# taipingeric/yolo-v4-tf.keras

Measured on AMD Instinct MI355X. Metric: images/sec end-to-end predict() at 608x608 batch 32; conv MFMA %peak, higher is better.
Workload: dtype bf16

## Files before the change

### yolo-v4-tf.keras_amd/csrc/resblock.hip

```cpp
#include <type_traits>

#include "conv_chain.h"

#ifndef RB_ABL
#define RB_ABL 0
#endif
#ifndef RB_RES_LDS
#define RB_RES_LDS 0
#endif
#ifndef RB_ST_AUX
#define RB_ST_AUX 0
#endif
#ifndef RB_LATE
#define RB_LATE 1
#endif

namespace y4 {

#ifdef RB_TRACE
__device__ unsigned long long rb_trace_buf[3 * 8 * 16];
#define RB_TR_WG 8
#define RB_TR_T0 1
#define RB_POINT(P)                                                                                         \
    do {                                                                                                    \
        __builtin_amdgcn_sched_barrier(0);                                                                  \
        if (tr_on) asm volatile("s_memtime %0" : "=s"(tr_t[P]));                                            \
        __builtin_amdgcn_sched_barrier(0);                                                                  \
    } while (0)
#else
#define RB_POINT(P)
#endif

constexpr int RB_ACT = (RB_ABL & 2) ? Y4_ACT_LEAKY : Y4_ACT_MISH;
constexpr int RB_T = 16, RB_H = RB_T + 2, RB_WAVES = 8;

template <int C, int TY = RB_T> struct RbGeom {
    static constexpr int HR = TY + 2;
    static constexpr int HROWS = HR * RB_H;
    static constexpr int NFA = HR + (2 * HR + 15) / 16;
    static constexpr int CPR = C / 8;
    static constexpr int ROWB = C * 2 + 16;
    static constexpr int XT_PIECES = (HROWS * (CPR + 1) + 63) / 64;
    static constexpr int NF = C / 16;
    static constexpr int KS1 = C / 32;
    static constexpr int STEP_BYTES = 2 * NF * 1024;
    static constexpr int P = KS1 / 2;
    static constexpr int NSTEPS = 10 * P;
    static constexpr int RING = 4;
    static constexpr int PPW = STEP_BYTES / 1024 / RB_WAVES;
    static constexpr int AFF_BYTES = 4 * C * 4;
    static constexpr int AFF_PAD = (AFF_BYTES + 1023) / 1024 * 1024;
    static constexpr int BLOB_BYTES = AFF_PAD + NSTEPS * STEP_BYTES;
    static constexpr int L_AFF = 0, L_RING = AFF_PAD, L_XT = L_RING + RING * STEP_BYTES;
    static constexpr int XT_SLACK = XT_PIECES * 1024 - HROWS * (CPR + 1) * 16;
    static constexpr int LDS = L_XT + XT_PIECES * 1024 + (XT_SLACK >= TOUCH_LDS ? 0 : 1024);
    static constexpr int L_TOUCH = LDS - TOUCH_LDS;
    static constexpr int WN = NF / 4, WM = RB_WAVES / WN, MREP = TY / WM;
    static_assert(C != 64 || 2 * LDS <= 160 * 1024, "C = 64: two workgroups per compute unit (resblock_dispatch)");
    static_assert(LDS <= 160 * 1024 && MREP >= 1 && MREP * WM == TY && PPW >= 1 && PPW * RB_WAVES * 1024 == STEP_BYTES && NFA <= 3 * RB_WAVES,
                  "resblock geometry");
};

struct ResBlockK {
    const char* in;
    char* out;
    const char* blob;
    int in_cstride, in_coff, out_cstride, out_coff;
    unsigned in_bytes, out_bytes;
    int N, S;
    int tiles_x, tiles_per_img, ntiles;
    int t_begin, t_end;
    int touch;
};

template <int DT, int C, int TY>
__global__ __launch_bounds__(64 * RB_WAVES, C == 64 ? 4 : 2) void resblock_kernel(const ResBlockK p) {
    using E = Elem<DT>;
    using G = RbGeom<C, TY>;
    constexpr int PARTS = RB_T / TY;
    constexpr int ROWB = G::ROWB, CPR = G::CPR, NF = G::NF, MREP = G::MREP;
    extern __shared__ __attribute__((aligned(16))) char smem[];
    const int tid = threadIdx.x, lane = tid & 63, wave = __builtin_amdgcn_readfirstlane(tid >> 6);
    const int q = lane & 15, g = lane >> 4;
    const int wm = wave / G::WN, wn = wave - wm * G::WN;
    const float* const aff = (const float*)(smem + G::L_AFF);
    char* const XT = smem + G::L_XT;
    char* const ring = smem + G::L_RING;

    const int GR = gridDim.x, xcd = blockIdx.x & 7, bi = blockIdx.x >> 3;
    const int nb_x = (GR - xcd + 7) >> 3;
    const int span = p.t_end - p.t_begin;
    const int t_lo = p.t_begin + (int)((int64_t)span * xcd / 8), t_hi = p.t_begin + (int)((int64_t)span * (xcd + 1) / 8);
    int t = t_lo + bi;
    auto locate = [&](int u, int& n, int& y_out0, int& tx) {
        const int full = u / PARTS, part = u - full * PARTS;
        n = full / p.tiles_per_img;
        const int rem = full - n * p.tiles_per_img, ty = rem / p.tiles_x;
        tx = rem - ty * p.tiles_x;
        y_out0 = ty * RB_T + part * TY;
    };

    const __amdgpu_buffer_rsrc_t rb = make_rsrc(p.blob, G::BLOB_BYTES);
    const __amdgpu_buffer_rsrc_t rs_in = make_rsrc(p.in, p.in_bytes), rs_out = make_rsrc(p.out, p.out_bytes);
    if (p.touch != 0) weight_touch(rb, smem + G::L_TOUCH, 0, G::BLOB_BYTES, wave, RB_WAVES, lane);
    for (int u = wave; u < G::AFF_PAD / 1024; u += RB_WAVES)
        buffer_load16_lds(rb, smem + __builtin_amdgcn_readfirstlane(u * 1024), u * 1024 + lane * 16, 0);
    auto stage_w = [&](int st) {
        char* const dst = ring + (st & (G::RING - 1)) * G::STEP_BYTES;
#pragma unroll
        for (int k = 0; k < G::PPW; ++k) {
            const int u = wave + k * RB_WAVES;
            buffer_load16_lds(rb, dst + __builtin_amdgcn_readfirstlane(u * 1024), G::AFF_PAD + u * 1024 + lane * 16, st * G::STEP_BYTES);
        }
    };
    auto load_x = [&](int tile) {
        int n, yo, tx;
        locate(tile, n, yo, tx);
        const int y0 = yo - 1, x0 = tx * RB_T - 1;
        constexpr int SPR = CPR + 1, DSLOT = RB_WAVES * 64, DHP = DSLOT / SPR, DCH = DSLOT % SPR, DHY = DHP / RB_H, DHX = DHP % RB_H;
        static_assert(DCH + SPR - 1 < 2 * SPR && DHX + RB_H < 2 * RB_H, "one carry per step");
        int slot0 = wave * 64 + lane;
        asm volatile("" : "+v"(slot0));
        const int hp0 = slot0 / SPR;
        int ch = slot0 - hp0 * SPR, hy = hp0 / RB_H;
        int hx = hp0 - hy * RB_H;
        const int pix_b = p.in_cstride * 2, row_b = p.S * pix_b;
        int off = (((n * p.S + y0) * p.S + x0) * p.in_cstride + p.in_coff) * 2 + hy * row_b + hx * pix_b + ch * 16;
        const int d_off = DHY * row_b + DHX * pix_b + DCH * 16, c_ch = pix_b - SPR * 16, c_hx = row_b - RB_H * pix_b;
#pragma unroll
        for (int k = 0; k * RB_WAVES < G::XT_PIECES; ++k) {
            const int u = wave + k * RB_WAVES;
            if (u < G::XT_PIECES) {
                const bool ok = ch < CPR && hy < G::HR && (unsigned)(y0 + hy) < (unsigned)p.S && (unsigned)(x0 + hx) < (unsigned)p.S;
                const int off_x = (RB_ABL & 128) ? (off & ~63) + (lane & 3) * 16 : off;
                buffer_load16_lds(rs_in, XT + __builtin_amdgcn_readfirstlane(u * 1024), ok ? off_x : (int)0x80000000, 0);
            }
            ch += DCH; hx += DHX; hy += DHY; off += d_off;
            if (ch >= SPR) { ch -= SPR; hx += 1; off += c_ch; }
            if (hx >= RB_H) { hx -= RB_H; hy += 1; off += c_hx; }
        }
    };
    if (t < t_hi) { load_x(t); stage_w(0); stage_w(1); stage_w(2); if (RB_LATE) stage_w(3); }

#ifdef RB_TRACE
    int tr_i = 0;
    unsigned long long tr_t[16] = {0, 0, 0, 0, 0, 0, 0, 0, 0, 0, 0, 0, 0, 0, 0, 0};
#endif
    for (; t < t_hi; t += nb_x) {
        int n, y_out0, tx;
        locate(t, n, y_out0, tx);
#ifdef RB_TRACE
        const bool tr_on = TY == RB_T && C == RB_TRACE && blockIdx.x == RB_TR_WG && tr_i >= RB_TR_T0 && tr_i < RB_TR_T0 + 3;
#endif
        RB_POINT(0);
        wait_vmcnt_then_barrier<0>();
        RB_POINT(1);

        u32x4 res[MREP][2];
        constexpr bool RES_LDS = RB_RES_LDS && (C == 128 || RB_RES_LDS > 1);
        if (RES_LDS) {
#pragma unroll
            for (int i = 0; i < MREP; ++i)
#pragma unroll
                for (int c = 0; c < 2; ++c)
                    res[i][c] = *(const u32x4*)(XT + ((wm * MREP + i + 1) * RB_H + q + 1) * ROWB + chunk_channel(wn * 64, c, g) * 2);
            asm volatile("s_waitcnt lgkmcnt(0)\n\ts_barrier" ::: "memory");
        }

        auto phase_a = [&](auto nfr_c) {
            constexpr int NFR = decltype(nfr_c)::value;
            char* row[NFR];
            bool inside[NFR];
#pragma unroll
            for (int k = 0; k < NFR; ++k) {
                const int f = wave + k * RB_WAVES;
                int hy, hx;
                if (f < G::HR) { hy = f; hx = 1 + q; }
                else { const int pp = min((f - G::HR) * 16 + q, 2 * G::HR - 1); hy = pp >> 1; hx = (pp & 1) * (RB_H - 1); }
                const int r = hy * RB_H + hx;
                row[k] = XT + r * ROWB;
                const int gy = y_out0 - 1 + hy, gx = tx * RB_T - 1 + hx;
                inside[k] = (unsigned)gy < (unsigned)p.S && (unsigned)gx < (unsigned)p.S;
            }
            f32x4 acc[NFR][NF];
#pragma unroll
            for (int k = 0; k < NFR; ++k)
#pragma unroll
                for (int j = 0; j < NF; ++j) acc[k][j] = f32x4{0.f, 0.f, 0.f, 0.f};
#pragma unroll
            for (int s = 0; s < G::KS1; ++s) {
                u32x4 xf[NFR], wf[NF];
#pragma unroll
                for (int k = 0; k < NFR; ++k) xf[k] = *(const u32x4*)(row[k] + (s * 4 + g) * 16);
#pragma unroll
                for (int j = 0; j < NF; ++j) wf[j] = *(const u32x4*)(ring + (s >> 1) * G::STEP_BYTES + (((s & 1) * NF + j) * 64 + lane) * 16);
#pragma unroll
                for (int k = 0; k < NFR; ++k)
#pragma unroll
                    for (int j = 0; j < NF; ++j) Mma<DT>::run(acc[k][j], wf[j], xf[k]);
            }
#pragma unroll
            for (int c = 0; c < NF / 2; ++c) {
                float sc[8], sh[8];
#pragma unroll
                for (int h = 0; h < 8; h += 4) {
                    const int ch = chunk_channel(0, c, g) + h;
                    const f32x4 s4 = *(const f32x4*)(aff + ch), h4 = *(const f32x4*)(aff + C + ch);
#pragma unroll
                    for (int e = 0; e < 4; ++e) { sc[h + e] = s4[e]; sh[h + e] = h4[e]; }
                }
#pragma unroll
                for (int k = 0; k < NFR; ++k) {
                    float v[8];
                    bn_act4<true, RB_ACT>(acc[k][2 * c], sc, sh, v);
                    bn_act4<true, RB_ACT>(acc[k][2 * c + 1], sc + 4, sh + 4, v + 4);
                    u32x4 pk;
                    E::store_chunk(&pk, v);
                    if (!inside[k]) pk = u32x4{0u, 0u, 0u, 0u};
                    *(u32x4*)(row[k] + (4 * c + g) * 16) = pk;
                }
            }
        };
        if (!(RB_ABL & 1)) {
            if (wave + 2 * RB_WAVES < G::NFA) phase_a(std::integral_constant<int, 3>{});
            else if (wave + RB_WAVES < G::NFA) phase_a(std::integral_constant<int, 2>{});
            else if (wave < G::NFA) phase_a(std::integral_constant<int, 1>{});
        }
        RB_POINT(2);
        asm volatile("s_waitcnt lgkmcnt(0)\n\ts_barrier" ::: "memory");
        RB_POINT(3);

        {
            int pix[MREP];
#pragma unroll
            for (int i = 0; i < MREP; ++i) {
                const int gy = y_out0 + wm * MREP + i, gx = tx * RB_T + q;
                pix[i] = gy < p.S && gx < p.S ? (n * p.S + gy) * p.S + gx : -1;
            }
            auto load_res = [&]() {
#pragma unroll
                for (int i = 0; i < MREP; ++i) {
                    const int o = pix[i] < 0 ? (int)0x80000000 : (pix[i] * p.in_cstride + p.in_coff) * 2;
#pragma unroll
                    for (int c = 0; c < 2; ++c) res[i][c] = buffer_load16(rs_in, o + chunk_channel(wn * 64, c, g) * 2);
                }
            };
            if (!RB_LATE && !RES_LDS) load_res();
            constexpr int S0 = G::NSTEPS - 4, RES_LOADS = RES_LDS ? 0 : 2 * MREP;
            f32x4 acc[MREP][4];
#pragma unroll
            for (int i = 0; i < MREP; ++i)
#pragma unroll
                for (int j = 0; j < 4; ++j) acc[i][j] = f32x4{0.f, 0.f, 0.f, 0.f};
#pragma unroll
            for (int st = RB_LATE ? 4 : 3; st <= G::P + 3; ++st) stage_w(st);
            const char* const xbase = XT + ((wm * MREP) * RB_H + q) * ROWB + g * 16;
            u32x4 xf[2][MREP], wf[2][4];
            auto read_frags = [&](int buf, int st, int kk) {
                if ((RB_ABL & 32) && st > G::P) return;
                const int ks = st - G::P;
                const int cb = ks / 9, tap = ks - cb * 9;
                const int ky = tap / 3, kx = tap - ky * 3;
                const char* const wst = ring + (st & (G::RING - 1)) * G::STEP_BYTES;
#pragma unroll
                for (int i = 0; i < MREP; ++i) {
                    xf[buf][i] = *(const u32x4*)(xbase + ((i + ky) * RB_H + kx) * ROWB + (cb * 8 + kk * 4) * 16);
                }
#pragma unroll
                for (int j = 0; j < 4; ++j) wf[buf][j] = *(const u32x4*)(wst + ((kk * NF + wn * 4 + j) * 64 + lane) * 16);
            };
            auto mma = [&](int buf) {
#pragma unroll
                for (int i = 0; i < MREP; ++i)
#pragma unroll
                    for (int j = 0; j < 4; ++j)
                        Mma<DT>::run(acc[i][j], wf[buf][j], xf[buf][i]);
            };
            RB_POINT(4);
            read_frags(0, G::P, 0);
#pragma unroll
            for (int st = G::P; st < G::NSTEPS; ++st) {
                if (st == G::P + 3 * G::P) RB_POINT(5);
                if (st == G::P + 6 * G::P) RB_POINT(6);
                if (RB_LATE && !RES_LDS && st == S0) load_res();
                read_frags(1, st, 1);
                __builtin_amdgcn_sched_barrier(0);
                mma(0);
                __builtin_amdgcn_sched_barrier(0);
                if (st + 1 < G::NSTEPS) {
                    constexpr int LAST = G::NSTEPS - 1;
                    const int younger = (st + 3 < LAST ? st + 3 : LAST) - (st + 1);
                    const int extra = RB_LATE && st >= S0 && st <= S0 + 2 ? RES_LOADS : 0;
                    static_assert(S0 > G::P && 2 * G::PPW + RES_LOADS < 64, "window of the residual's loads");
                    if (RB_ABL & 64) asm volatile("s_waitcnt vmcnt(0)" ::: "memory");
                    else wait_vmcnt_lgkm_then_barrier_n<2 * G::PPW + RES_LOADS>(younger == 0 ? 0 : (younger >= 2 ? 2 : 1) * G::PPW + extra);
                    if (!(RB_ABL & 4) && st + 4 < G::NSTEPS) stage_w(st + 4);
                    read_frags(0, st + 1, 0);
                    __builtin_amdgcn_sched_barrier(0);
                }
                mma(1);
                __builtin_amdgcn_sched_barrier(0);
            }
            RB_POINT(7);
            asm volatile("s_waitcnt lgkmcnt(0)\n\ts_barrier" ::: "memory");
            RB_POINT(8);
            if constexpr (RB_LATE && !RES_LDS) {
#pragma unroll
                for (int i = 0; i < MREP; ++i)
#pragma unroll
                    for (int c = 0; c < 2; ++c) asm volatile("" : "+v"(res[i][c]));
            }
            const bool more = t + nb_x < t_hi;
            if (more) { if (!(RB_ABL & 8)) load_x(t + nb_x); stage_w(0); stage_w(1); stage_w(2); if (RB_LATE) stage_w(3); }
            RB_POINT(9);
            float sc3[16], sh3[16];
#pragma unroll
            for (int c = 0; c < 2; ++c)
#pragma unroll
                for (int h = 0; h < 8; h += 4) {
                    const int ch = chunk_channel(wn * 64, c, g) + h;
                    const f32x4 s4 = *(const f32x4*)(aff + 2 * C + ch), h4 = *(const f32x4*)(aff + 3 * C + ch);
#pragma unroll
                    for (int e = 0; e < 4; ++e) { sc3[c * 8 + h + e] = s4[e]; sh3[c * 8 + h + e] = h4[e]; }
                }
#pragma unroll
            for (int i = 0; i < MREP; ++i) {
                float v[16];
#pragma unroll
                for (int j = 0; j < 4; ++j) bn_act4<true, RB_ACT>(acc[i][j], sc3 + j * 4, sh3 + j * 4, v + j * 4);
                const int o = pix[i] < 0 ? (int)0x80000000 : (pix[i] * p.out_cstride + p.out_coff) * 2;
#pragma unroll
                for (int c = 0; c < 2; ++c) {
                    float rv[8];
                    E::load_chunk(&res[i][c], rv);
#pragma unroll
                    for (int e = 0; e < 8; ++e) v[c * 8 + e] += rv[e];
                    u32x4 pk;
                    E::store_chunk(&pk, v + c * 8);
                    if (!(RB_ABL & 16) || pk[0] == 0x12345678u) buffer_store16<RB_ST_AUX>(rs_out, pk, o + chunk_channel(wn * 64, c, g) * 2);
                }
            }
        }
        RB_POINT(10);
#ifdef RB_TRACE
        if (tr_on && lane == 0) {
#pragma unroll
            for (int k = 0; k < 11; ++k) rb_trace_buf[((tr_i - RB_TR_T0) * 8 + wave) * 16 + k] = tr_t[k];
        }
        ++tr_i;
#endif
    }
}

#ifdef RB_TRACE
}
extern "C" int y4_rb_trace_read(unsigned long long* dst) {
    return (int)hipMemcpyFromSymbol(dst, HIP_SYMBOL(y4::rb_trace_buf), sizeof(unsigned long long) * 3 * 8 * 16);
}
namespace y4 {
#endif

bool resblock_supported(int dtype, int c) { return dtype != Y4_F32 && (c == 128 || c == 64); }
size_t resblock_blob_bytes(int c) { return c == 128 ? RbGeom<128>::BLOB_BYTES : RbGeom<64>::BLOB_BYTES; }

template <int DT, int C, int TY>
static int resblock_run(const ResBlockK& k, int slots, hipStream_t stream) {
    int grid = slots;
    const int span = k.t_end - k.t_begin;
    if (grid > ((span + 7) & ~7)) grid = (span + 7) & ~7;
    if (grid < 8) grid = 8;
    constexpr int lds = RbGeom<C, TY>::LDS;
    static PerDeviceOnce once;
    if (const uint64_t bit = once.due()) {
        Y4_CHECK_HIP(hipFuncSetAttribute((const void*)resblock_kernel<DT, C, TY>, hipFuncAttributeMaxDynamicSharedMemorySize, lds));
        once.mark(bit);
    }
    hipLaunchKernelGGL((resblock_kernel<DT, C, TY>), dim3(grid), dim3(64 * RB_WAVES), lds, stream, k);
    Y4_CHECK_HIP(hipGetLastError());
    return Y4_OK;
}

static bool rb_parts_enabled() {
    static const bool on = [] { const char* e = getenv("Y4_RB_PARTS"); return !(e && e[0] == '0'); }();
    return on;
}

template <int DT, int C>
static int resblock_dispatch(ResBlockK& k, hipStream_t stream) {
    static int n_cus[64] = {0};
    int dev = 0;
    Y4_CHECK_HIP(hipGetDevice(&dev));
    if (n_cus[dev & 63] == 0) {
        int v = 0;
        Y4_CHECK_HIP(hipDeviceGetAttribute(&v, hipDeviceAttributeMultiprocessorCount, dev));
        n_cus[dev & 63] = v > 0 ? v : 256;
    }
    const int slots = (n_cus[dev & 63] & ~7) * (C == 64 ? 2 : 1);
    constexpr int MAXP = C == 128 ? 4 : 2;
    const int full = k.ntiles / slots * slots, rem = k.ntiles - full;
    int parts = 1;
    if (rb_parts_enabled() && rem > 0)
        for (int pp = 2; pp <= MAXP; pp *= 2)
            if (rem * pp <= slots) parts = pp;
    if (parts == 1) {
        k.t_begin = 0; k.t_end = k.ntiles;
        return resblock_run<DT, C, RB_T>(k, slots, stream);
    }
    if (full > 0) {
        k.t_begin = 0; k.t_end = full;
        if (int r = resblock_run<DT, C, RB_T>(k, slots, stream)) return r;
    }
    k.t_begin = full * parts; k.t_end = k.ntiles * parts;
    if (parts == 2) return resblock_run<DT, C, RB_T / 2>(k, slots, stream);
    if constexpr (MAXP >= 4) return resblock_run<DT, C, RB_T / 4>(k, slots, stream);
    return Y4_EINVAL;
}

int resblock_launch(int dtype, int c, const void* in, int n, int side, int in_cstride, int in_coff, const void* blob, void* out,
                    int out_cstride, int out_coff, hipStream_t stream) {
    Y4_REQUIRE(resblock_supported(dtype, c), Y4_EINVAL, "resblock: dtype %d / %d channels not supported", dtype, c);
    Y4_REQUIRE(in && blob && out && n > 0 && side > 0, Y4_EINVAL, "resblock: null pointer / empty batch");
    Y4_REQUIRE(in_cstride % 8 == 0 && in_coff % 8 == 0 && out_cstride % 8 == 0 && out_coff % 8 == 0, Y4_EINVAL,
               "resblock: views not 16-byte aligned");
    const int64_t in_bytes = (int64_t)n * side * side * in_cstride * 2;
    const int64_t out_bytes = (int64_t)n * side * side * out_cstride * 2;
    Y4_REQUIRE(in_bytes < (1ll << 31) && out_bytes < (1ll << 31), Y4_EINVAL,
               "resblock: input (%lld B) or output (%lld B) exceeds the 2 GiB buffer-descriptor range", (long long)in_bytes, (long long)out_bytes);
    ResBlockK k{};
    k.in = (const char*)in; k.out = (char*)out; k.blob = (const char*)blob;
    k.in_cstride = in_cstride; k.in_coff = in_coff; k.out_cstride = out_cstride; k.out_coff = out_coff;
    k.in_bytes = (unsigned)in_bytes; k.out_bytes = (unsigned)out_bytes;
    k.N = n; k.S = side;
    k.touch = weight_touch_enabled() ? 1 : 0;
    k.tiles_x = (side + RB_T - 1) / RB_T; k.tiles_per_img = k.tiles_x * k.tiles_x; k.ntiles = n * k.tiles_per_img;
    if (c == 128) return dtype == Y4_BF16 ? resblock_dispatch<Y4_BF16, 128>(k, stream) : resblock_dispatch<Y4_F16, 128>(k, stream);
    return dtype == Y4_BF16 ? resblock_dispatch<Y4_BF16, 64>(k, stream) : resblock_dispatch<Y4_F16, 64>(k, stream);
}

template <int DT>
__global__ void rb_pack_frag_kernel(const float* __restrict__ w, typename Elem<DT>::type* __restrict__ out, int cout, int cin, int kk) {
    const int nrep = cout / 16, cbs = cin / 32, total = cout * cin * kk;
    for (int idx = blockIdx.x * blockDim.x + threadIdx.x; idx < total; idx += gridDim.x * blockDim.x) {
        const int e = idx & 7, lane = (idx >> 3) & 63, r = idx >> 9;
        const int j = r % nrep, s = r / nrep;
        const int step = s >> 1, cb64 = step / kk, tap = step - cb64 * kk, cb = cb64 * 2 + (s & 1);
        const int i = lane & 15, gg = lane >> 4;
        const int ch = ((j >> 1) * 4 + (i >> 2)) * 8 + (j & 1) * 4 + (i & 3);
        const int ci = 32 * cb + 8 * gg + e;
        out[idx] = Elem<DT>::st(w[((int64_t)ch * cin + ci) * kk + tap]);
    }
}
__global__ void rb_affine_kernel(const float* s1, const float* h1, const float* s3, const float* h3, float* dst, int c) {
    const int i = blockIdx.x * blockDim.x + threadIdx.x;
    if (i < c) { dst[i] = s1[i]; dst[c + i] = h1[i]; dst[2 * c + i] = s3[i]; dst[3 * c + i] = h3[i]; }
}

int pack_resblock(int dtype, int c, const float* w1, const float* scale1, const float* shift1, const float* w3, const float* scale3,
                  const float* shift3, void* blob, hipStream_t stream) {
    Y4_REQUIRE(resblock_supported(dtype, c) && w1 && w3 && scale1 && shift1 && scale3 && shift3 && blob, Y4_EINVAL, "pack_resblock: bad argument");
    const int w1_bytes = c * c * 2, aff_pad = (4 * c * 4 + 1023) / 1024 * 1024;
    char* b = (char*)blob;
    if (dtype == Y4_BF16) {
        hipLaunchKernelGGL(rb_pack_frag_kernel<Y4_BF16>, dim3((c * c + 255) / 256), dim3(256), 0, stream, w1, (uint16_t*)(b + aff_pad), c, c, 1);
        hipLaunchKernelGGL(rb_pack_frag_kernel<Y4_BF16>, dim3((9 * c * c + 255) / 256), dim3(256), 0, stream, w3, (uint16_t*)(b + aff_pad + w1_bytes), c, c, 9);
    } else {
        hipLaunchKernelGGL(rb_pack_frag_kernel<Y4_F16>, dim3((c * c + 255) / 256), dim3(256), 0, stream, w1, (_Float16*)(b + aff_pad), c, c, 1);
        hipLaunchKernelGGL(rb_pack_frag_kernel<Y4_F16>, dim3((9 * c * c + 255) / 256), dim3(256), 0, stream, w3, (_Float16*)(b + aff_pad + w1_bytes), c, c, 9);
    }
    hipLaunchKernelGGL(rb_affine_kernel, dim3(1), dim3(128), 0, stream, scale1, shift1, scale3, shift3, (float*)b, c);
    Y4_CHECK_HIP(hipGetLastError());
    return Y4_OK;
}

}
```

Baseline: 5923.

## Rewrite fused resblock kernel with 19x19 tiles, 4 waves, resident weights

Rewrites the fused 1x1+3x3 residual-block kernel. Tiles grow to 19x19 outputs with 4 waves and one workgroup per CU. The 1x1 weights, and for C=64 also the 3x3 weights, now stay resident in LDS. For C=128 the 3x3 weights stream from global memory into a register ring instead of an LDS staging ring with barriers. It also drops the tile-split tail dispatch, the weight-touch prefetch, the ablation flags and the trace instrumentation. The intent is to cut per-step barriers and LDS weight traffic and to lower halo overhead per output, at the cost of lower occupancy and more register pressure.

```diff
diff --git a/yolo-v4-tf.keras_amd/csrc/resblock.hip b/yolo-v4-tf.keras_amd/csrc/resblock.hip
--- a/yolo-v4-tf.keras_amd/csrc/resblock.hip
+++ b/yolo-v4-tf.keras_amd/csrc/resblock.hip
@@ -2,63 +2,55 @@
 
 #include "conv_chain.h"
 
-#ifndef RB_ABL
-#define RB_ABL 0
+#ifndef RB_WD
+#define RB_WD 4
 #endif
-#ifndef RB_RES_LDS
-#define RB_RES_LDS 0
-#endif
-#ifndef RB_ST_AUX
-#define RB_ST_AUX 0
-#endif
-#ifndef RB_LATE
-#define RB_LATE 1
-#endif
 
 namespace y4 {
 
-#ifdef RB_TRACE
-__device__ unsigned long long rb_trace_buf[3 * 8 * 16];
-#define RB_TR_WG 8
-#define RB_TR_T0 1
-#define RB_POINT(P)                                                                                         \
-    do {                                                                                                    \
-        __builtin_amdgcn_sched_barrier(0);                                                                  \
-        if (tr_on) asm volatile("s_memtime %0" : "=s"(tr_t[P]));                                            \
-        __builtin_amdgcn_sched_barrier(0);                                                                  \
-    } while (0)
-#else
-#define RB_POINT(P)
-#endif
-
-constexpr int RB_ACT = (RB_ABL & 2) ? Y4_ACT_LEAKY : Y4_ACT_MISH;
-constexpr int RB_T = 16, RB_H = RB_T + 2, RB_WAVES = 8;
-
-template <int C, int TY = RB_T> struct RbGeom {
-    static constexpr int HR = TY + 2;
-    static constexpr int HROWS = HR * RB_H;
-    static constexpr int NFA = HR + (2 * HR + 15) / 16;
+template <int I, int N, class F> __device__ __forceinline__ void rb_static_for(F&& f) {
+    if constexpr (I < N) {
+        f(std::integral_constant<int, I>{});
+        rb_static_for<I + 1, N>(f);
+    }
+}
+
+__device__ __forceinline__ u32x4 buffer_load16_so(__amdgpu_buffer_rsrc_t rsrc, int voffset, int soffset) {
+    return __builtin_amdgcn_raw_buffer_load_b128(rsrc, voffset, soffset, 0);
+}
+
+constexpr int RB_T = 19, RB_H = RB_T + 2, RB_WAVES = 4;
+constexpr int RB_HP = RB_H * RB_H;
+constexpr int RB_NFA = (RB_HP + 15) / 16;
+constexpr int RB_NPO = RB_T * RB_T;
+constexpr int RB_NFO = (RB_NPO + 15) / 16;
+
+template <int C> struct RbGeom {
+    static constexpr int NF = C / 16;
+    static constexpr int KS1 = C / 32, KS3 = 9 * KS1;
     static constexpr int CPR = C / 8;
-    static constexpr int ROWB = C * 2 + 16;
-    static constexpr int XT_PIECES = (HROWS * (CPR + 1) + 63) / 64;
-    static constexpr int NF = C / 16;
-    static constexpr int KS1 = C / 32;
-    static constexpr int STEP_BYTES = 2 * NF * 1024;
-    static constexpr int P = KS1 / 2;
-    static constexpr int NSTEPS = 10 * P;
-    static constexpr int RING = 4;
-    static constexpr int PPW = STEP_BYTES / 1024 / RB_WAVES;
+    static constexpr int SPR = CPR + 2, ROWB = SPR * 16;
+    static constexpr int EXTRA = C == 64 ? 192 : 0, RSTR = RB_H * ROWB + EXTRA;
+    static constexpr int RSPR = RSTR / 16;
+    static constexpr int XT_SLOTS = RB_H * RSPR + (RB_NFA * 16 - RB_HP) * SPR;
     static constexpr int AFF_BYTES = 4 * C * 4;
     static constexpr int AFF_PAD = (AFF_BYTES + 1023) / 1024 * 1024;
-    static constexpr int BLOB_BYTES = AFF_PAD + NSTEPS * STEP_BYTES;
-    static constexpr int L_AFF = 0, L_RING = AFF_PAD, L_XT = L_RING + RING * STEP_BYTES;
-    static constexpr int XT_SLACK = XT_PIECES * 1024 - HROWS * (CPR + 1) * 16;
-    static constexpr int LDS = L_XT + XT_PIECES * 1024 + (XT_SLACK >= TOUCH_LDS ? 0 : 1024);
-    static constexpr int L_TOUCH = LDS - TOUCH_LDS;
-    static constexpr int WN = NF / 4, WM = RB_WAVES / WN, MREP = TY / WM;
-    static_assert(C != 64 || 2 * LDS <= 160 * 1024, "C = 64: two workgroups per compute unit (resblock_dispatch)");
-    static_assert(LDS <= 160 * 1024 && MREP >= 1 && MREP * WM == TY && PPW >= 1 && PPW * RB_WAVES * 1024 == STEP_BYTES && NFA <= 3 * RB_WAVES,
-                  "resblock geometry");
+    static constexpr int W1_BYTES = C * C * 2, W3_BYTES = 9 * C * C * 2;
+    static constexpr int BLOB_BYTES = AFF_PAD + W1_BYTES + W3_BYTES;
+    static constexpr bool W3_LDS = C == 64;
+    static constexpr int L_W1 = AFF_PAD, L_W3 = AFF_PAD + W1_BYTES;
+    static constexpr int L_XT = AFF_PAD + W1_BYTES + (W3_LDS ? W3_BYTES : 0);
+    static constexpr int RES_PIECES = L_XT / 1024;
+    static constexpr int XT_PIECES = (XT_SLOTS + 63) / 64;
+    static constexpr int LDS = L_XT + XT_PIECES * 1024;
+    static constexpr int WF = C == 128 ? 2 : 4, WP = C == 128 ? RB_NFO : (RB_NFO + RB_WAVES - 1) / RB_WAVES;
+    static constexpr int WD = W3_LDS ? 2 : RB_WD;
+    static constexpr int S_RES = C == 128 ? KS3 - 12 : 0;
+    static constexpr int NST = WP * (WF / 2);
+    static_assert(L_XT % 1024 == 0 && EXTRA % 16 == 0 && LDS <= 160 * 1024, "resblock LDS layout");
+    static_assert(WF * (C == 128 ? RB_WAVES : 1) == NF && WP * (C == 128 ? 1 : RB_WAVES) >= RB_NFO && RB_NFA % RB_WAVES == 0,
+                  "resblock wave split");
+    static_assert(WD >= 2 && WD <= KS3, "weight ring depth");
 };
 
 struct ResBlockK {
@@ -69,133 +61,95 @@
     unsigned in_bytes, out_bytes;
     int N, S;
     int tiles_x, tiles_per_img, ntiles;
-    int t_begin, t_end;
-    int touch;
 };
 
-template <int DT, int C, int TY>
-__global__ __launch_bounds__(64 * RB_WAVES, C == 64 ? 4 : 2) void resblock_kernel(const ResBlockK p) {
+template <int DT, int C>
+__global__ __launch_bounds__(64 * RB_WAVES, 1) void resblock_kernel(const ResBlockK p) {
     using E = Elem<DT>;
-    using G = RbGeom<C, TY>;
-    constexpr int PARTS = RB_T / TY;
-    constexpr int ROWB = G::ROWB, CPR = G::CPR, NF = G::NF, MREP = G::MREP;
+    using G = RbGeom<C>;
+    constexpr int ROWB = G::ROWB, RSTR = G::RSTR, CPR = G::CPR, SPR = G::SPR, NF = G::NF, WF = G::WF, WP = G::WP, WD = G::WD;
     extern __shared__ __attribute__((aligned(16))) char smem[];
     const int tid = threadIdx.x, lane = tid & 63, wave = __builtin_amdgcn_readfirstlane(tid >> 6);
     const int q = lane & 15, g = lane >> 4;
-    const int wm = wave / G::WN, wn = wave - wm * G::WN;
-    const float* const aff = (const float*)(smem + G::L_AFF);
+    const float* const aff = (const float*)smem;
+    const char* const W1 = smem + G::L_W1;
+    const char* const W3L = smem + G::L_W3;
     char* const XT = smem + G::L_XT;
-    char* const ring = smem + G::L_RING;
 
     const int GR = gridDim.x, xcd = blockIdx.x & 7, bi = blockIdx.x >> 3;
     const int nb_x = (GR - xcd + 7) >> 3;
-    const int span = p.t_end - p.t_begin;
-    const int t_lo = p.t_begin + (int)((int64_t)span * xcd / 8), t_hi = p.t_begin + (int)((int64_t)span * (xcd + 1) / 8);
+    const int t_lo = (int)((int64_t)p.ntiles * xcd / 8), t_hi = (int)((int64_t)p.ntiles * (xcd + 1) / 8);
     int t = t_lo + bi;
-    auto locate = [&](int u, int& n, int& y_out0, int& tx) {
-        const int full = u / PARTS, part = u - full * PARTS;
-        n = full / p.tiles_per_img;
-        const int rem = full - n * p.tiles_per_img, ty = rem / p.tiles_x;
-        tx = rem - ty * p.tiles_x;
-        y_out0 = ty * RB_T + part * TY;
+    auto locate = [&](int u, int& n, int& y0, int& x0) {
+        n = u / p.tiles_per_img;
+        const int rem = u - n * p.tiles_per_img, ty = rem / p.tiles_x;
+        y0 = ty * RB_T;
+        x0 = (rem - ty * p.tiles_x) * RB_T;
     };
 
     const __amdgpu_buffer_rsrc_t rb = make_rsrc(p.blob, G::BLOB_BYTES);
     const __amdgpu_buffer_rsrc_t rs_in = make_rsrc(p.in, p.in_bytes), rs_out = make_rsrc(p.out, p.out_bytes);
-    if (p.touch != 0) weight_touch(rb, smem + G::L_TOUCH, 0, G::BLOB_BYTES, wave, RB_WAVES, lane);
-    for (int u = wave; u < G::AFF_PAD / 1024; u += RB_WAVES)
+    for (int u = wave; u < G::RES_PIECES; u += RB_WAVES)
         buffer_load16_lds(rb, smem + __builtin_amdgcn_readfirstlane(u * 1024), u * 1024 + lane * 16, 0);
-    auto stage_w = [&](int st) {
-        char* const dst = ring + (st & (G::RING - 1)) * G::STEP_BYTES;
-#pragma unroll
-        for (int k = 0; k < G::PPW; ++k) {
-            const int u = wave + k * RB_WAVES;
-            buffer_load16_lds(rb, dst + __builtin_amdgcn_readfirstlane(u * 1024), G::AFF_PAD + u * 1024 + lane * 16, st * G::STEP_BYTES);
+    auto load_x = [&](int tile) {
+        int n, y0, x0;
+        locate(tile, n, y0, x0);
+        const int pix_b = p.in_cstride * 2;
+        const int base = (((n * p.S + y0 - 1) * p.S + x0 - 1) * p.in_cstride + p.in_coff) * 2;
+        for (int u = wave; u < G::XT_PIECES; u += RB_WAVES) {
+            const int slot = u * 64 + lane, hy = slot / G::RSPR, r = slot - hy * G::RSPR, hx = r / SPR, ch = r - hx * SPR;
+            const bool ok = ch < CPR && hx < RB_H && hy < RB_H && (unsigned)(y0 - 1 + hy) < (unsigned)p.S && (unsigned)(x0 - 1 + hx) < (unsigned)p.S;
+            buffer_load16_lds(rs_in, XT + __builtin_amdgcn_readfirstlane(u * 1024), ok ? base + (hy * p.S + hx) * pix_b + ch * 16 : (int)0x80000000, 0);
         }
     };
-    auto load_x = [&](int tile) {
-        int n, yo, tx;
-        locate(tile, n, yo, tx);
-        const int y0 = yo - 1, x0 = tx * RB_T - 1;
-        constexpr int SPR = CPR + 1, DSLOT = RB_WAVES * 64, DHP = DSLOT / SPR, DCH = DSLOT % SPR, DHY = DHP / RB_H, DHX = DHP % RB_H;
-        static_assert(DCH + SPR - 1 < 2 * SPR && DHX + RB_H < 2 * RB_H, "one carry per step");
-        int slot0 = wave * 64 + lane;
-        asm volatile("" : "+v"(slot0));
-        const int hp0 = slot0 / SPR;
-        int ch = slot0 - hp0 * SPR, hy = hp0 / RB_H;
-        int hx = hp0 - hy * RB_H;
-        const int pix_b = p.in_cstride * 2, row_b = p.S * pix_b;
-        int off = (((n * p.S + y0) * p.S + x0) * p.in_cstride + p.in_coff) * 2 + hy * row_b + hx * pix_b + ch * 16;
-        const int d_off = DHY * row_b + DHX * pix_b + DCH * 16, c_ch = pix_b - SPR * 16, c_hx = row_b - RB_H * pix_b;
-#pragma unroll
-        for (int k = 0; k * RB_WAVES < G::XT_PIECES; ++k) {
-            const int u = wave + k * RB_WAVES;
-            if (u < G::XT_PIECES) {
-                const bool ok = ch < CPR && hy < G::HR && (unsigned)(y0 + hy) < (unsigned)p.S && (unsigned)(x0 + hx) < (unsigned)p.S;
-                const int off_x = (RB_ABL & 128) ? (off & ~63) + (lane & 3) * 16 : off;
-                buffer_load16_lds(rs_in, XT + __builtin_amdgcn_readfirstlane(u * 1024), ok ? off_x : (int)0x80000000, 0);
-            }
-            ch += DCH; hx += DHX; hy += DHY; off += d_off;
-            if (ch >= SPR) { ch -= SPR; hx += 1; off += c_ch; }
-            if (hx >= RB_H) { hx -= RB_H; hy += 1; off += c_hx; }
+    if (t < t_hi) load_x(t);
+
+    const int wfrag0 = G::W3_LDS ? 0 : wave * WF;
+    const int w3_off = G::L_W3 + (wfrag0 * 64 + lane) * 16;
+    auto fetch_w = [&](u32x4 (&w)[WF], int s) {
+#pragma unroll
+        for (int j = 0; j < WF; ++j) {
+            if constexpr (G::W3_LDS) w[j] = *(const u32x4*)(smem + w3_off + (s * NF + j) * 1024);
+            else w[j] = buffer_load16_so(rb, w3_off, (s * NF + j) * 1024);
         }
     };
-    if (t < t_hi) { load_x(t); stage_w(0); stage_w(1); stage_w(2); if (RB_LATE) stage_w(3); }
-
-#ifdef RB_TRACE
-    int tr_i = 0;
-    unsigned long long tr_t[16] = {0, 0, 0, 0, 0, 0, 0, 0, 0, 0, 0, 0, 0, 0, 0, 0};
-#endif
-    for (; t < t_hi; t += nb_x) {
-        int n, y_out0, tx;
-        locate(t, n, y_out0, tx);
-#ifdef RB_TRACE
-        const bool tr_on = TY == RB_T && C == RB_TRACE && blockIdx.x == RB_TR_WG && tr_i >= RB_TR_T0 && tr_i < RB_TR_T0 + 3;
-#endif
-        RB_POINT(0);
-        wait_vmcnt_then_barrier<0>();
-        RB_POINT(1);
-
-        u32x4 res[MREP][2];
-        constexpr bool RES_LDS = RB_RES_LDS && (C == 128 || RB_RES_LDS > 1);
-        if (RES_LDS) {
-#pragma unroll
-            for (int i = 0; i < MREP; ++i)
-#pragma unroll
-                for (int c = 0; c < 2; ++c)
-                    res[i][c] = *(const u32x4*)(XT + ((wm * MREP + i + 1) * RB_H + q + 1) * ROWB + chunk_channel(wn * 64, c, g) * 2);
-            asm volatile("s_waitcnt lgkmcnt(0)\n\ts_barrier" ::: "memory");
-        }
-
-        auto phase_a = [&](auto nfr_c) {
-            constexpr int NFR = decltype(nfr_c)::value;
-            char* row[NFR];
-            bool inside[NFR];
-#pragma unroll
-            for (int k = 0; k < NFR; ++k) {
-                const int f = wave + k * RB_WAVES;
-                int hy, hx;
-                if (f < G::HR) { hy = f; hx = 1 + q; }
-                else { const int pp = min((f - G::HR) * 16 + q, 2 * G::HR - 1); hy = pp >> 1; hx = (pp & 1) * (RB_H - 1); }
-                const int r = hy * RB_H + hx;
-                row[k] = XT + r * ROWB;
-                const int gy = y_out0 - 1 + hy, gx = tx * RB_T - 1 + hx;
-                inside[k] = (unsigned)gy < (unsigned)p.S && (unsigned)gx < (unsigned)p.S;
-            }
-            f32x4 acc[NFR][NF];
-#pragma unroll
-            for (int k = 0; k < NFR; ++k)
+    const int pf0 = G::W3_LDS ? wave * WP : 0;
+
+    for (bool first = true; t < t_hi; t += nb_x, first = false) {
+        int n, y0, x0;
+        locate(t, n, y0, x0);
+        if (first) wait_vmcnt_then_barrier<0>();
+        else wait_vmcnt_then_barrier<G::NST>();
+        u32x4 wr[WD][WF];
+#pragma unroll
+        for (int s = 0; s < WD - 1; ++s) fetch_w(wr[s], s);
+
+        {
+            constexpr int NA = RB_NFA / RB_WAVES;
+            char* row[NA];
+            bool inside[NA];
+            int qa = q;
+            asm volatile("" : "+v"(qa));
+#pragma unroll
+            for (int k = 0; k < NA; ++k) {
+                const int hp = (wave + k * RB_WAVES) * 16 + qa, hy = hp / RB_H, hx = hp - hy * RB_H;
+                row[k] = XT + hy * RSTR + hx * ROWB;
+                inside[k] = hp < RB_HP && (unsigned)(y0 - 1 + hy) < (unsigned)p.S && (unsigned)(x0 - 1 + hx) < (unsigned)p.S;
+            }
+            f32x4 acc[NA][NF];
+#pragma unroll
+            for (int k = 0; k < NA; ++k)
 #pragma unroll
                 for (int j = 0; j < NF; ++j) acc[k][j] = f32x4{0.f, 0.f, 0.f, 0.f};
 #pragma unroll
             for (int s = 0; s < G::KS1; ++s) {
-                u32x4 xf[NFR], wf[NF];
-#pragma unroll
-                for (int k = 0; k < NFR; ++k) xf[k] = *(const u32x4*)(row[k] + (s * 4 + g) * 16);
-#pragma unroll
-                for (int j = 0; j < NF; ++j) wf[j] = *(const u32x4*)(ring + (s >> 1) * G::STEP_BYTES + (((s & 1) * NF + j) * 64 + lane) * 16);
-#pragma unroll
-                for (int k = 0; k < NFR; ++k)
+                u32x4 xf[NA], wf[NF];
+#pragma unroll
+                for (int k = 0; k < NA; ++k) xf[k] = *(const u32x4*)(row[k] + (s * 4 + g) * 16);
+#pragma unroll
+                for (int j = 0; j < NF; ++j) wf[j] = *(const u32x4*)(W1 + ((s * NF + j) * 64 + lane) * 16);
+#pragma unroll
+                for (int k = 0; k < NA; ++k)
 #pragma unroll
                     for (int j = 0; j < NF; ++j) Mma<DT>::run(acc[k][j], wf[j], xf[k]);
             }
@@ -210,183 +164,103 @@
                     for (int e = 0; e < 4; ++e) { sc[h + e] = s4[e]; sh[h + e] = h4[e]; }
                 }
 #pragma unroll
-                for (int k = 0; k < NFR; ++k) {
+                for (int k = 0; k < NA; ++k) {
                     float v[8];
-                    bn_act4<true, RB_ACT>(acc[k][2 * c], sc, sh, v);
-                    bn_act4<true, RB_ACT>(acc[k][2 * c + 1], sc + 4, sh + 4, v + 4);
+                    bn_act4<true, Y4_ACT_MISH>(acc[k][2 * c], sc, sh, v);
+                    bn_act4<true, Y4_ACT_MISH>(acc[k][2 * c + 1], sc + 4, sh + 4, v + 4);
                     u32x4 pk;
                     E::store_chunk(&pk, v);
                     if (!inside[k]) pk = u32x4{0u, 0u, 0u, 0u};
                     *(u32x4*)(row[k] + (4 * c + g) * 16) = pk;
                 }
             }
+        }
+        asm volatile("s_waitcnt lgkmcnt(0)\n\ts_barrier" ::: "memory");
+
+        int xrow[WP];
+#pragma unroll
+        for (int i = 0; i < WP; ++i) {
+            const int pp = (pf0 + i) * 16 + q, pc = min(pp, RB_NPO - 1), oy = pc / RB_T, ox = pc - oy * RB_T;
+            xrow[i] = oy * RSTR + ox * ROWB + g * 16;
+        }
+        auto pix = [&](int i) {
+            int qq = q;
+            asm volatile("" : "+v"(qq));
+            const int pp = (pf0 + i) * 16 + qq, oy = pp / RB_T, ox = pp - oy * RB_T, gy = y0 + oy, gx = x0 + ox;
+            return ((pp < RB_NPO) & (gy < p.S) & (gx < p.S)) ? (n * p.S + gy) * p.S + gx : -1;
         };
-        if (!(RB_ABL & 1)) {
-            if (wave + 2 * RB_WAVES < G::NFA) phase_a(std::integral_constant<int, 3>{});
-            else if (wave + RB_WAVES < G::NFA) phase_a(std::integral_constant<int, 2>{});
-            else if (wave < G::NFA) phase_a(std::integral_constant<int, 1>{});
-        }
-        RB_POINT(2);
+        auto xoff = [](int s) constexpr {
+            const int cb = s / 18, r = s - cb * 18, tap = r >> 1, ky = tap / 3, kx = tap - ky * 3;
+            return ky * RSTR + kx * ROWB + (cb * 8 + (r & 1) * 4) * 16;
+        };
+        f32x4 acc[WP][WF];
+#pragma unroll
+        for (int i = 0; i < WP; ++i)
+#pragma unroll
+            for (int j = 0; j < WF; ++j) acc[i][j] = f32x4{0.f, 0.f, 0.f, 0.f};
+        u32x4 xf[WP];
+#pragma unroll
+        for (int i = 0; i < WP; ++i) xf[i] = *(const u32x4*)(XT + xrow[i]);
+        constexpr int NRES = WF / 2;
+        u32x4 res[WP][NRES];
+        rb_static_for<0, G::KS3>([&](auto sc) __attribute__((always_inline)) {
+            constexpr int s = decltype(sc)::value;
+            if constexpr (s + WD - 1 < G::KS3) fetch_w(wr[(s + WD - 1) % WD], s + WD - 1);
+            if constexpr (s == G::S_RES) {
+#pragma unroll
+                for (int i = 0; i < WP; ++i) {
+                    const int pi = pix(i), o = pi < 0 ? (int)0x80000000 : (pi * p.in_cstride + p.in_coff) * 2;
+#pragma unroll
+                    for (int c = 0; c < NRES; ++c) res[i][c] = buffer_load16(rs_in, o + chunk_channel(0, wfrag0 / 2 + c, g) * 2);
+                }
+            }
+            const u32x4(&w)[WF] = wr[s % WD];
+#pragma unroll
+            for (int i = 0; i < WP; ++i) {
+#pragma unroll
+                for (int j = 0; j < WF; ++j) Mma<DT>::run(acc[i][j], w[j], xf[i]);
+                if constexpr (s + 1 < G::KS3) xf[i] = *(const u32x4*)(XT + xrow[i] + xoff(s + 1));
+            }
+            __builtin_amdgcn_sched_barrier(0);
+        });
         asm volatile("s_waitcnt lgkmcnt(0)\n\ts_barrier" ::: "memory");
-        RB_POINT(3);
-
-        {
-            int pix[MREP];
-#pragma unroll
-            for (int i = 0; i < MREP; ++i) {
-                const int gy = y_out0 + wm * MREP + i, gx = tx * RB_T + q;
-                pix[i] = gy < p.S && gx < p.S ? (n * p.S + gy) * p.S + gx : -1;
-            }
-            auto load_res = [&]() {
-#pragma unroll
-                for (int i = 0; i < MREP; ++i) {
-                    const int o = pix[i] < 0 ? (int)0x80000000 : (pix[i] * p.in_cstride + p.in_coff) * 2;
-#pragma unroll
-                    for (int c = 0; c < 2; ++c) res[i][c] = buffer_load16(rs_in, o + chunk_channel(wn * 64, c, g) * 2);
-                }
-            };
-            if (!RB_LATE && !RES_LDS) load_res();
-            constexpr int S0 = G::NSTEPS - 4, RES_LOADS = RES_LDS ? 0 : 2 * MREP;
-            f32x4 acc[MREP][4];
-#pragma unroll
-            for (int i = 0; i < MREP; ++i)
-#pragma unroll
-                for (int j = 0; j < 4; ++j) acc[i][j] = f32x4{0.f, 0.f, 0.f, 0.f};
-#pragma unroll
-            for (int st = RB_LATE ? 4 : 3; st <= G::P + 3; ++st) stage_w(st);
-            const char* const xbase = XT + ((wm * MREP) * RB_H + q) * ROWB + g * 16;
-            u32x4 xf[2][MREP], wf[2][4];
-            auto read_frags = [&](int buf, int st, int kk) {
-                if ((RB_ABL & 32) && st > G::P) return;
-                const int ks = st - G::P;
-                const int cb = ks / 9, tap = ks - cb * 9;
-                const int ky = tap / 3, kx = tap - ky * 3;
-                const char* const wst = ring + (st & (G::RING - 1)) * G::STEP_BYTES;
-#pragma unroll
-                for (int i = 0; i < MREP; ++i) {
-                    xf[buf][i] = *(const u32x4*)(xbase + ((i + ky) * RB_H + kx) * ROWB + (cb * 8 + kk * 4) * 16);
-                }
-#pragma unroll
-                for (int j = 0; j < 4; ++j) wf[buf][j] = *(const u32x4*)(wst + ((kk * NF + wn * 4 + j) * 64 + lane) * 16);
-            };
-            auto mma = [&](int buf) {
-#pragma unroll
-                for (int i = 0; i < MREP; ++i)
-#pragma unroll
-                    for (int j = 0; j < 4; ++j)
-                        Mma<DT>::run(acc[i][j], wf[buf][j], xf[buf][i]);
-            };
-            RB_POINT(4);
-            read_frags(0, G::P, 0);
-#pragma unroll
-            for (int st = G::P; st < G::NSTEPS; ++st) {
-                if (st == G::P + 3 * G::P) RB_POINT(5);
-                if (st == G::P + 6 * G::P) RB_POINT(6);
-                if (RB_LATE && !RES_LDS && st == S0) load_res();
-                read_frags(1, st, 1);
-                __builtin_amdgcn_sched_barrier(0);
-                mma(0);
-                __builtin_amdgcn_sched_barrier(0);
-                if (st + 1 < G::NSTEPS) {
-                    constexpr int LAST = G::NSTEPS - 1;
-                    const int younger = (st + 3 < LAST ? st + 3 : LAST) - (st + 1);
-                    const int extra = RB_LATE && st >= S0 && st <= S0 + 2 ? RES_LOADS : 0;
-                    static_assert(S0 > G::P && 2 * G::PPW + RES_LOADS < 64, "window of the residual's loads");
-                    if (RB_ABL & 64) asm volatile("s_waitcnt vmcnt(0)" ::: "memory");
-                    else wait_vmcnt_lgkm_then_barrier_n<2 * G::PPW + RES_LOADS>(younger == 0 ? 0 : (younger >= 2 ? 2 : 1) * G::PPW + extra);
-                    if (!(RB_ABL & 4) && st + 4 < G::NSTEPS) stage_w(st + 4);
-                    read_frags(0, st + 1, 0);
-                    __builtin_amdgcn_sched_barrier(0);
-                }
-                mma(1);
-                __builtin_amdgcn_sched_barrier(0);
-            }
-            RB_POINT(7);
-            asm volatile("s_waitcnt lgkmcnt(0)\n\ts_barrier" ::: "memory");
-            RB_POINT(8);
-            if constexpr (RB_LATE && !RES_LDS) {
-#pragma unroll
-                for (int i = 0; i < MREP; ++i)
-#pragma unroll
-                    for (int c = 0; c < 2; ++c) asm volatile("" : "+v"(res[i][c]));
-            }
-            const bool more = t + nb_x < t_hi;
-            if (more) { if (!(RB_ABL & 8)) load_x(t + nb_x); stage_w(0); stage_w(1); stage_w(2); if (RB_LATE) stage_w(3); }
-            RB_POINT(9);
-            float sc3[16], sh3[16];
-#pragma unroll
-            for (int c = 0; c < 2; ++c)
-#pragma unroll
-                for (int h = 0; h < 8; h += 4) {
-                    const int ch = chunk_channel(wn * 64, c, g) + h;
-                    const f32x4 s4 = *(const f32x4*)(aff + 2 * C + ch), h4 = *(const f32x4*)(aff + 3 * C + ch);
-#pragma unroll
-                    for (int e = 0; e < 4; ++e) { sc3[c * 8 + h + e] = s4[e]; sh3[c * 8 + h + e] = h4[e]; }
-                }
-#pragma unroll
-            for (int i = 0; i < MREP; ++i) {
-                float v[16];
-#pragma unroll
-                for (int j = 0; j < 4; ++j) bn_act4<true, RB_ACT>(acc[i][j], sc3 + j * 4, sh3 + j * 4, v + j * 4);
-                const int o = pix[i] < 0 ? (int)0x80000000 : (pix[i] * p.out_cstride + p.out_coff) * 2;
-#pragma unroll
-                for (int c = 0; c < 2; ++c) {
-                    float rv[8];
-                    E::load_chunk(&res[i][c], rv);
-#pragma unroll
-                    for (int e = 0; e < 8; ++e) v[c * 8 + e] += rv[e];
-                    u32x4 pk;
-                    E::store_chunk(&pk, v + c * 8);
-                    if (!(RB_ABL & 16) || pk[0] == 0x12345678u) buffer_store16<RB_ST_AUX>(rs_out, pk, o + chunk_channel(wn * 64, c, g) * 2);
-                }
-            }
-        }
-        RB_POINT(10);
-#ifdef RB_TRACE
-        if (tr_on && lane == 0) {
-#pragma unroll
-            for (int k = 0; k < 11; ++k) rb_trace_buf[((tr_i - RB_TR_T0) * 8 + wave) * 16 + k] = tr_t[k];
-        }
-        ++tr_i;
-#endif
-    }
-}
-
-#ifdef RB_TRACE
-}
-extern "C" int y4_rb_trace_read(unsigned long long* dst) {
-    return (int)hipMemcpyFromSymbol(dst, HIP_SYMBOL(y4::rb_trace_buf), sizeof(unsigned long long) * 3 * 8 * 16);
-}
-namespace y4 {
-#endif
+#pragma unroll
+        for (int i = 0; i < WP; ++i)
+#pragma unroll
+            for (int c = 0; c < NRES; ++c) asm volatile("" : "+v"(res[i][c]));
+        if (t + nb_x < t_hi) load_x(t + nb_x);
+#pragma unroll
+        for (int c = 0; c < NRES; ++c) {
+            const int ch = chunk_channel(0, wfrag0 / 2 + c, g);
+            float sc3[8], sh3[8];
+#pragma unroll
+            for (int h = 0; h < 8; h += 4) {
+                const f32x4 s4 = *(const f32x4*)(aff + 2 * C + ch + h), h4 = *(const f32x4*)(aff + 3 * C + ch + h);
+#pragma unroll
+                for (int e = 0; e < 4; ++e) { sc3[h + e] = s4[e]; sh3[h + e] = h4[e]; }
+            }
+#pragma unroll
+            for (int i = 0; i < WP; ++i) {
+                float v[8], rv[8];
+                bn_act4<true, Y4_ACT_MISH>(acc[i][2 * c], sc3, sh3, v);
+                bn_act4<true, Y4_ACT_MISH>(acc[i][2 * c + 1], sc3 + 4, sh3 + 4, v + 4);
+                E::load_chunk(&res[i][c], rv);
+#pragma unroll
+                for (int e = 0; e < 8; ++e) v[e] += rv[e];
+                u32x4 pk;
+                E::store_chunk(&pk, v);
+                const int pi = pix(i), o = pi < 0 ? (int)0x80000000 : (pi * p.out_cstride + p.out_coff) * 2;
+                buffer_store16(rs_out, pk, o + ch * 2);
+            }
+        }
+    }
+}
 
 bool resblock_supported(int dtype, int c) { return dtype != Y4_F32 && (c == 128 || c == 64); }
 size_t resblock_blob_bytes(int c) { return c == 128 ? RbGeom<128>::BLOB_BYTES : RbGeom<64>::BLOB_BYTES; }
 
-template <int DT, int C, int TY>
-static int resblock_run(const ResBlockK& k, int slots, hipStream_t stream) {
-    int grid = slots;
-    const int span = k.t_end - k.t_begin;
-    if (grid > ((span + 7) & ~7)) grid = (span + 7) & ~7;
-    if (grid < 8) grid = 8;
-    constexpr int lds = RbGeom<C, TY>::LDS;
-    static PerDeviceOnce once;
-    if (const uint64_t bit = once.due()) {
-        Y4_CHECK_HIP(hipFuncSetAttribute((const void*)resblock_kernel<DT, C, TY>, hipFuncAttributeMaxDynamicSharedMemorySize, lds));
-        once.mark(bit);
-    }
-    hipLaunchKernelGGL((resblock_kernel<DT, C, TY>), dim3(grid), dim3(64 * RB_WAVES), lds, stream, k);
-    Y4_CHECK_HIP(hipGetLastError());
-    return Y4_OK;
-}
-
-static bool rb_parts_enabled() {
-    static const bool on = [] { const char* e = getenv("Y4_RB_PARTS"); return !(e && e[0] == '0'); }();
-    return on;
-}
-
 template <int DT, int C>
-static int resblock_dispatch(ResBlockK& k, hipStream_t stream) {
+static int resblock_run(const ResBlockK& k, hipStream_t stream) {
     static int n_cus[64] = {0};
     int dev = 0;
     Y4_CHECK_HIP(hipGetDevice(&dev));
@@ -395,25 +269,18 @@
         Y4_CHECK_HIP(hipDeviceGetAttribute(&v, hipDeviceAttributeMultiprocessorCount, dev));
         n_cus[dev & 63] = v > 0 ? v : 256;
     }
-    const int slots = (n_cus[dev & 63] & ~7) * (C == 64 ? 2 : 1);
-    constexpr int MAXP = C == 128 ? 4 : 2;
-    const int full = k.ntiles / slots * slots, rem = k.ntiles - full;
-    int parts = 1;
-    if (rb_parts_enabled() && rem > 0)
-        for (int pp = 2; pp <= MAXP; pp *= 2)
-            if (rem * pp <= slots) parts = pp;
-    if (parts == 1) {
-        k.t_begin = 0; k.t_end = k.ntiles;
-        return resblock_run<DT, C, RB_T>(k, slots, stream);
-    }
-    if (full > 0) {
-        k.t_begin = 0; k.t_end = full;
-        if (int r = resblock_run<DT, C, RB_T>(k, slots, stream)) return r;
-    }
-    k.t_begin = full * parts; k.t_end = k.ntiles * parts;
-    if (parts == 2) return resblock_run<DT, C, RB_T / 2>(k, slots, stream);
-    if constexpr (MAXP >= 4) return resblock_run<DT, C, RB_T / 4>(k, slots, stream);
-    return Y4_EINVAL;
+    int grid = n_cus[dev & 63] & ~7;
+    if (grid > ((k.ntiles + 7) & ~7)) grid = (k.ntiles + 7) & ~7;
+    if (grid < 8) grid = 8;
+    constexpr int lds = RbGeom<C>::LDS;
+    static PerDeviceOnce once;
+    if (const uint64_t bit = once.due()) {
+        Y4_CHECK_HIP(hipFuncSetAttribute((const void*)resblock_kernel<DT, C>, hipFuncAttributeMaxDynamicSharedMemorySize, lds));
+        once.mark(bit);
+    }
+    hipLaunchKernelGGL((resblock_kernel<DT, C>), dim3(grid), dim3(64 * RB_WAVES), lds, stream, k);
+    Y4_CHECK_HIP(hipGetLastError());
+    return Y4_OK;
 }
 
 int resblock_launch(int dtype, int c, const void* in, int n, int side, int in_cstride, int in_coff, const void* blob, void* out,
@@ -431,10 +298,9 @@
     k.in_cstride = in_cstride; k.in_coff = in_coff; k.out_cstride = out_cstride; k.out_coff = out_coff;
     k.in_bytes = (unsigned)in_bytes; k.out_bytes = (unsigned)out_bytes;
     k.N = n; k.S = side;
-    k.touch = weight_touch_enabled() ? 1 : 0;
     k.tiles_x = (side + RB_T - 1) / RB_T; k.tiles_per_img = k.tiles_x * k.tiles_x; k.ntiles = n * k.tiles_per_img;
-    if (c == 128) return dtype == Y4_BF16 ? resblock_dispatch<Y4_BF16, 128>(k, stream) : resblock_dispatch<Y4_F16, 128>(k, stream);
-    return dtype == Y4_BF16 ? resblock_dispatch<Y4_BF16, 64>(k, stream) : resblock_dispatch<Y4_F16, 64>(k, stream);
+    if (c == 128) return dtype == Y4_BF16 ? resblock_run<Y4_BF16, 128>(k, stream) : resblock_run<Y4_F16, 128>(k, stream);
+    return dtype == Y4_BF16 ? resblock_run<Y4_BF16, 64>(k, stream) : resblock_run<Y4_F16, 64>(k, stream);
 }
 
 template <int DT>
```

After: 5972, median of 6. No clear change (+0.8%).
